# xmindflow/cenet

Measured on AMD Instinct MI355X. Metric: training images/sec (224x224, 4-class), higher is better.
Workload: dtype bf16

## Files before the change

### cenet_amd/csrc/common.h

```cpp
#pragma once

#ifdef CENET_HOSTSIM_BUILD
#include "hipsim.h"
#else
#include <hip/hip_runtime.h>
#include <cstdint>
#include <cstring>
typedef float f32x4 __attribute__((ext_vector_type(4)));
typedef float f32x16 __attribute__((ext_vector_type(16)));
typedef short bf16x8 __attribute__((ext_vector_type(8)));
#define CENET_LAUNCH(kernel, grid, block, stream, ...) \
  hipLaunchKernelGGL(kernel, (grid), (block), 0, (stream), __VA_ARGS__)
#endif

#define CENET_WAVE 64

struct cenet_bid {
  int x, y, z;
};
__device__ __forceinline__ cenet_bid cenet_xcd_block() {
  const int gx = gridDim.x, gy = gridDim.y;
  const int T = gx * gy * (int)gridDim.z;
  int L = blockIdx.x + gx * (blockIdx.y + gy * blockIdx.z);
  if (T >= 64) {
    const int per = T >> 3, rem = T & 7, xcd = L & 7, idx = L >> 3;
    L = xcd * per + (xcd < rem ? xcd : rem) + idx;
  }
  cenet_bid b;
  b.x = L % gx;
  const int t = L / gx;
  b.y = t % gy;
  b.z = t / gy;
  return b;
}

#ifdef CENET_HOSTSIM_BUILD
static const unsigned ring_zero16[4] = {0, 0, 0, 0};
#else
__device__ __attribute__((aligned(16))) const unsigned ring_zero16[4] = {0, 0, 0, 0};
#endif

__device__ __forceinline__ void ring_glds16(const void* gsrc, unsigned char* wave_base, int lane) {
#ifdef CENET_HOSTSIM_BUILD
  memcpy(wave_base + 16 * lane, gsrc, 16);
#else
  (void)lane;
  __builtin_amdgcn_global_load_lds((const __attribute__((address_space(1))) unsigned*)gsrc,
                                   (__attribute__((address_space(3))) unsigned*)wave_base, 16, 0, 0);
#endif
}

template <int N>
__device__ __forceinline__ void ring_wait_vm() {
#ifndef CENET_HOSTSIM_BUILD
  asm volatile("s_waitcnt vmcnt(%0)" ::"n"(N) : "memory");
#endif
}
__device__ __forceinline__ void ring_barrier() {
#ifdef CENET_HOSTSIM_BUILD
  __syncthreads();
#else
  asm volatile("s_barrier" ::: "memory");
#endif
}


#ifdef CENET_HOSTSIM_BUILD
__device__ __forceinline__ unsigned cenet_f2bf(float f) {
  unsigned u;
  memcpy(&u, &f, 4);
  u += 0x7FFFu + ((u >> 16) & 1u);
  return u >> 16;
}
__device__ __forceinline__ unsigned cenet_pack_bf2(float lo, float hi) { return cenet_f2bf(lo) | (cenet_f2bf(hi) << 16); }
#else
typedef __bf16 cenet_bf2_t __attribute__((ext_vector_type(2)));
__device__ __forceinline__ unsigned cenet_pack_bf2(float lo, float hi) {
  cenet_bf2_t v = {(__bf16)lo, (__bf16)hi};
  unsigned u;
  memcpy(&u, &v, 4);
  return u;
}
__device__ __forceinline__ unsigned cenet_f2bf(float f) { return cenet_pack_bf2(f, 0.f); }
#endif

typedef unsigned short bf16_t;
__device__ __forceinline__ float cenet_bf2f(unsigned h) {
  unsigned u = h << 16;
  float f;
  memcpy(&f, &u, 4);
  return f;
}
__device__ __forceinline__ float ldf(const float* p) { return *p; }
__device__ __forceinline__ float ldf(const bf16_t* p) { return cenet_bf2f(*p); }
__device__ __forceinline__ void stf(float* p, float v) { *p = v; }
__device__ __forceinline__ void stf(bf16_t* p, float v) { *p = (bf16_t)cenet_f2bf(v); }
struct f4 {
  float v[4];
};
__device__ __forceinline__ f4 ld4(const float* p) {
  f4 r;
  memcpy(r.v, p, 16);
  return r;
}
__device__ __forceinline__ f4 ld4(const bf16_t* p) {
  unsigned u[2];
  memcpy(u, p, 8);
  f4 r;
  r.v[0] = cenet_bf2f(u[0] & 0xFFFFu);
  r.v[1] = cenet_bf2f(u[0] >> 16);
  r.v[2] = cenet_bf2f(u[1] & 0xFFFFu);
  r.v[3] = cenet_bf2f(u[1] >> 16);
  return r;
}
__device__ __forceinline__ void st4(float* p, const f4& r) { memcpy(p, r.v, 16); }
// ... 244 lines not shown
```

### cenet_amd/csrc/gemm.hip

```cpp
#include "gemm_ring.h"
#include <cstdio>
#include <cstdlib>

static void pick_tile(int M, int N, int nbatch, int splits, int* bm, int* bn) {
  int m = M >= 96 ? 128 : (M >= 48 ? 64 : 32);
  int n = N >= 96 ? 128 : 64;
  if (m == 32) n = N >= 192 ? 256 : 64;
  long blocks = (long)cdiv(M, m) * cdiv(N, n) * nbatch * splits;
  if (blocks < 256 && m > 32) {
    int m2 = m > 64 ? 64 : m, n2 = n > 64 ? 64 : n;
    if (M >= 48) {
      m = m2;
      n = n2;
    }
  }
  *bm = m;
  *bn = n;
}

static thread_local char g_last_kernel[96] = "";
extern "C" const char* cenet_gemm_last_kernel(void) { return g_last_kernel; }
static inline const char* tf(bool b) { return b ? "true" : "false"; }

#ifdef CENET_RING_STAMPS
static unsigned long long* g_stamp_buf = nullptr;
static int g_stamp_n = 0;
extern "C" int cenet_ring_stamps(unsigned long long* buf, int n) {
  if (buf != nullptr && n <= 0) return CENET_EINVAL;
  g_stamp_buf = buf;
  g_stamp_n = buf ? n : 0;
  return CENET_OK;
}
#endif

template <typename GT>
__global__ __launch_bounds__(256) void gemm_asum_kernel(const GT* __restrict__ A, long sr, long sc, long skb, int M, int K, int nkb,
                                                       float* __restrict__ asum) {
  __shared__ float red[16];
  if (sr == 1 && sc != 1) {
    const int m = blockIdx.x * 256 + threadIdx.x;
    if (m >= M) return;
    const long total = (long)nkb * K;
    float s = 0.f;
    for (long e = blockIdx.y; e < total; e += gridDim.y) {
      const long kb = e / K, k = e - kb * K;
      s += ldf(A + kb * skb + k * sc + m);
    }
    atomicAdd(&asum[m], s);
  } else {
    const int m = blockIdx.x;
    const long total = (long)nkb * K;
    float s = 0.f;
    for (long e = blockIdx.y * 256 + threadIdx.x; e < total; e += (long)gridDim.y * 256) {
      const long kb = e / K, k = e - kb * K;
      s += ldf(A + kb * skb + (long)m * sr + k * sc);
    }
    s = block_sum(s, red);
    if (threadIdx.x == 0) atomicAdd(&asum[m], s);
  }
}
extern "C" int cenet_col_sum_acc_f32(const float* a, float* out_acc, long R, int C, hipStream_t stream);
extern "C" int cenet_col_sum_acc_bf16(const bf16_t* a, float* out_acc, long R, int C, hipStream_t stream);
extern "C" int cenet_chan_dot_acc_f32(const float* a, long sab, const float* b, long sbb, float* out_acc, int B, int C, int HW,
                                      hipStream_t stream);
extern "C" int cenet_chan_dot_acc_bf16(const bf16_t* a, long sab, const bf16_t* b, long sbb, float* out_acc, int B, int C, int HW,
                                       hipStream_t stream);

template <typename GT>
static void launch_asum(const cenet_mat_t* A, int M, int K, int nkb, float* asum, hipStream_t stream) {
  if (A->sr == 1 && A->sc == M && nkb == 1) {
    if (sizeof(GT) == 2) cenet_col_sum_acc_bf16((const bf16_t*)A->ptr, asum, K, M, stream);
    else cenet_col_sum_acc_f32((const float*)A->ptr, asum, K, M, stream);
    return;
  }
  if (A->sc == 1 && A->sr == K && (nkb == 1 || A->skb >= (long)M * K)) {
// ... 84 lines not shown
      g.b_end = (const unsigned short*)B->ptr + b_last;
      if (lda < 0 || ldb < 0 || a_last < 8 || b_last < 8) akf = bkf = -1;
    } else {
      akf = bkf = -1;
    }
  }
  static const bool ring_off = getenv("CENET_GEMM_NO_RING") != nullptr;
  const bool ring = !ring_off && akf >= 0 && bkf >= 0 && !E->cmode && E->act == ACT_NONE && M >= 48 && N >= 48;
  if (ring) {
    static const char* force = getenv("CENET_RING_TILE");
    if (force) {
      sscanf(force, "%dx%d", &bm, &bn);
    } else if (E->atomic) {
      bm = bn = 64;
      if ((long)K * nkb >= 4096 && (long)M * N >= 131072) {
        if (N >= 128) bn = 128;
        else bm = 128;
      }
    } else {
      bm = M >= 96 ? 128 : 64;
      bn = N >= 96 ? 128 : 64;
      const long want = K >= 320 ? 400 : 256;
      auto wgs = [&](int a, int b) { return (long)cdiv(M, a) * cdiv(N, b) * nbatch; };
      if (wgs(bm, bn) < want && bm == 128 && bn == 128) (M >= N ? bm : bn) = 64;
      if (wgs(bm, bn) < want && (bm == 128 || bn == 128)) bm = bn = 64;
      static const char* fb = getenv("CENET_RING_TILE_BATCHED");
      if (fb && nbatch >= 8) sscanf(fb, "%dx%d", &bm, &bn);
    }
  }
  const int kstep = ring ? 64 : BK;
  if (E->atomic && !E->cmode && splits > 1) {
    const long tiles = (long)cdiv(M, bm) * cdiv(N, bn) * nbatch;
    const long iters = (long)nkb * cdiv(K, kstep);
    const double t_iter = ring ? 0.5 : ((B->mode == 1) ? 2.0 : 0.9);
    const double t_atom = (double)tiles * bm * bn * 4.0 / 1.3e6;
    long s = (long)(__builtin_sqrt((double)iters * t_iter / t_atom) + 0.5);
    const long slots = (bm * bn >= 128 * 128) ? 512 : (bm * bn >= 128 * 64 ? 768 : 1024);
    if (s * tiles > slots) s = slots / tiles;
    if (s > iters / 2) s = iters / 2;
    if (s > 256) s = 256;
    if (s < 1) s = 1;
    static const char* sm = getenv("CENET_RING_SPLIT_MUL");
    if (ring && sm) {
      s = (long)(s * atof(sm) + 0.5);
      if (s > iters / 2) s = iters / 2;
      if (s < 1) s = 1;
    }
    splits = (int)s;
    g.splits = splits;
  }
  const bool im = B->mode != 0;
  int rc;
  static const bool stream_off = getenv("CENET_GEMM_NO_STREAM") != nullptr;
  const bool rstream = ring && !stream_off && !E->atomic && nkb == 1 && splits <= 1 && !g.ring_unal && (K == 64 || K == 128) &&
                       (long)cdiv(M, 64) * cdiv(N, 64) * nbatch >= 768;
  if (rstream) {
    snprintf(g_last_kernel, sizeof g_last_kernel, "gemm_ring_stream_kernel<%s, %s, %s, %d>", tf(akf), tf(bkf), tf(swap), K / 64);
    rc = akf ? (bkf ? cenet_gemm_launch_ring_kk(g, 0, 0, nbatch, swap, stream) : cenet_gemm_launch_ring_kr(g, 0, 0, nbatch, swap, stream))
             : (bkf ? cenet_gemm_launch_ring_rk(g, 0, 0, nbatch, swap, stream) : cenet_gemm_launch_ring_rr(g, 0, 0, nbatch, swap, stream));
  } else if (ring) {
    snprintf(g_last_kernel, sizeof g_last_kernel, "gemm_ring_kernel<%s, %s, %d, %d, %d, %s>", tf(akf), tf(bkf), bm, bn,
             bm == 128 && bn == 128 ? 2 : (bm == 64 && bn == 64 ? 4 : 3), tf(swap));
    rc = akf ? (bkf ? cenet_gemm_launch_ring_kk(g, bm, bn, nbatch, swap, stream) : cenet_gemm_launch_ring_kr(g, bm, bn, nbatch, swap, stream))
             : (bkf ? cenet_gemm_launch_ring_rk(g, bm, bn, nbatch, swap, stream) : cenet_gemm_launch_ring_rr(g, bm, bn, nbatch, swap, stream));
  } else if (bf) {
    if (E->asum) {
      launch_asum<unsigned short>(A, M, K, nkb, E->asum, stream);
      g.E.asum = nullptr;
    }
    const long kchunk = ((long)nkb * K) / (splits > 0 ? splits : 1);
    const bool k64 = !im && K >= 128 && kchunk >= 128 && bm <= 64 && bn == 64;
    snprintf(g_last_kernel, sizeof g_last_kernel, "gemm_kernel<unsigned short, %d, %d, %s, %s, %d>", bm, bn, tf(im), tf(swap),
             k64 ? 64 : 32);
    rc = im ? cenet_gemm_launch_bf16_im2col(g, bm, bn, nbatch, swap, stream)
            : (k64 ? cenet_gemm_launch_bf16_plain_k64(g, bm, bn, nbatch, swap, stream)
                   : cenet_gemm_launch_bf16_plain(g, bm, bn, nbatch, swap, stream));
  }
  else {
    if (E->asum) {
      launch_asum<float>(A, M, K, nkb, E->asum, stream);
      g.E.asum = nullptr;
    }
    snprintf(g_last_kernel, sizeof g_last_kernel, "gemm_kernel<float, %d, %d, %s, %s, 32>", bm, bn, tf(im), tf(swap));
    rc = im ? cenet_gemm_launch_f32_im2col(g, bm, bn, nbatch, swap, stream) : cenet_gemm_launch_f32_plain(g, bm, bn, nbatch, swap, stream);
  }
  if (rc != CENET_OK) return rc;
  CENET_CHECK_LAUNCH();
  return CENET_OK;
}

extern "C" int cenet_gemm_f32(const cenet_mat_t* A, const cenet_mat_t* B, const cenet_epi_t* E, int M, int N, int K,
                              int nbatch, int nb_inner, int nkb, int splits, hipStream_t stream) {
  return gemm_dispatch(A, B, E, M, N, K, nbatch, nb_inner, nkb, splits, 4, stream);
}
extern "C" int cenet_gemm_bf16(const cenet_mat_t* A, const cenet_mat_t* B, const cenet_epi_t* E, int M, int N, int K,
                               int nbatch, int nb_inner, int nkb, int splits, hipStream_t stream) {
  return gemm_dispatch(A, B, E, M, N, K, nbatch, nb_inner, nkb, splits, 2, stream);
}
```

### cenet_amd/csrc/gemm_core.h

```cpp
#pragma once
#include "common.h"
#include "../../include/cenet_hip.h"

struct GemmArgs {
  cenet_mat_t A, B;
  cenet_epi_t E;
  int M, N, K, nkb, splits, nb_inner;
  int avec, bvec, cvec;
  int cvec8;
  int apair, bpair;
  int ring_unal;
  const void *a_end, *b_end;
#ifdef CENET_RING_STAMPS
  unsigned long long* stamps;
  int stamp_n;
#endif
};

__device__ __forceinline__ unsigned f2bf_bits(float f) { return cenet_f2bf(f); }
__device__ __forceinline__ unsigned pack_bf2(float lo, float hi) { return cenet_pack_bf2(lo, hi); }

template <typename OpT, int KT> struct OpTraits { static constexpr int PITCH = KT + (sizeof(OpT) == 4 ? 4 : 8); };
#define BK 32

// ... 381 lines not shown
            const int row = SWAP ? rbase : rbase + r, col = SWAP ? cbase + r : cbase;
            if (row < g.M && col < g.N) {
              float t = v[r];
              if (E.bias) t += E.bias[E.bias_on_row ? row : col];
              t *= bsr > 0 ? E.bscale[row / bsr] : bs;
              if (Rb) t += ldf(Rb + (long)row * E.srr + (long)col * E.src);
              stf(Cb + (long)row * E.scr + (long)col * E.scc, t);
            }
          }
        }
      }
    return;
  }
  for (int f = 0; f < MI * NJ; ++f) {
    f32x4 t4 = acc[0][0];
#pragma unroll
    for (int i = 0; i < MI; ++i)
#pragma unroll
      for (int j = 0; j < NJ; ++j)
        if (f == i * NJ + j) t4 = acc[i][j];
    const int rbase = rwave + (f / NJ) * 16, cbase = cwave + (f % NJ) * 16;
#pragma unroll
    for (int r = 0; r < 4; ++r) {
      const int row = SWAP ? rbase : rbase + r, col = SWAP ? cbase + r : cbase;
      if (row < g.M && col < g.N) {
        float v = t4[r] * E.alpha;
        if (E.cmode) {
          const int kkw = E.cKH * E.cKW;
          const int ci = row / kkw, rem = row - ci * kkw;
          const int ky = rem / E.cKW, kx = rem - ky * E.cKW;
          const int py = col / E.cPw, px = col - py * E.cPw;
          const int iy = py * E.cstride - E.cpad + ky, ix = px * E.cstride - E.cpad + kx;
          if (iy >= 0 && iy < E.cHs && ix >= 0 && ix < E.cWs) {
            const long o = (long)ci * E.csci + (long)iy * E.csy + (long)ix * E.csx;
            if (E.atomic) atomicAdd(&Cf[o], v);
            else stf(&Cb[o], v);
          }
        } else if (E.atomic == 2) {
          Cf[(long)row * E.scr + (long)col * E.scc] = v;
        } else if (E.atomic) {
          atomicAdd(&Cf[(long)row * E.scr + (long)col * E.scc], v);
        } else {
          if (E.bias) v += E.bias[E.bias_on_row ? row : col];
          v = act_fwd(E.act, v, E.slope);
          v *= bsr > 0 ? E.bscale[row / bsr] : bs;
          if (Rb) v += ldf(Rb + (long)row * E.srr + (long)col * E.src);
          stf(&Cb[(long)row * E.scr + (long)col * E.scc], v);
        }
      }
    }
  }
}

template <typename OpT, int BM, int BN, bool B_IM2COL, bool SWAP, int KT>
__global__ __launch_bounds__(256, (BM * BN >= 128 * 128 ? 2 : 1)) void gemm_kernel(GemmArgs g) {
  static_assert(KT == 32 || (KT == 64 && !B_IM2COL), "K step: 32, or 64 for plain operands");
  constexpr int P = OpTraits<OpT, KT>::PITCH;
  constexpr bool BF = (sizeof(OpT) == 2);
  constexpr int MI = BM / 32, NJ = BN / 32;
  constexpr int NA = BM * KT / 256, NB = BN * KT / 256;
  typedef OpT GT;
  __shared__ __attribute__((aligned(16))) OpT As[BM * P];
  __shared__ __attribute__((aligned(16))) OpT Bs[BN * P];
  __shared__ KEntry ntab[B_IM2COL ? BN : 1];
  __shared__ float cstrip[SWAP ? 1 : 4 * 16 * (BN / 2 + 1)];

  const int tid = threadIdx.x, wave = tid >> 6, lane = tid & 63;
  const int wm = wave >> 1, wn = wave & 1;
  int bx, by, bz;
  {
    const int gx = gridDim.x, gy = gridDim.y;
    const int T = gx * gy * (int)gridDim.z;
    int L = blockIdx.x + gx * (blockIdx.y + gy * blockIdx.z);
    if (T >= 64) {
      const int per = T >> 3, rem = T & 7, xcd = L & 7, idx = L >> 3;
      L = xcd * per + (xcd < rem ? xcd : rem) + idx;
    }
    bx = L % gx;
    const int t = L / gx;
    by = t % gy;
    bz = t / gy;
  }
  const int batch = bz / g.splits, split = bz - batch * g.splits;
  const int bo = batch / g.nb_inner, bi = batch - bo * g.nb_inner;
  const int m0 = by * BM, n0 = bx * BN;

  f32x4 acc[MI][NJ];
#pragma unroll
  for (int i = 0; i < MI; ++i)
#pragma unroll
    for (int j = 0; j < NJ; ++j) acc[i][j] = f32x4{0.f, 0.f, 0.f, 0.f};

  const int ktiles = (g.K + KT - 1) / KT;
  const int total = g.nkb * ktiles;
  const int chunk = (total + g.splits - 1) / g.splits;
  const int it0 = split * chunk;
  const int it1 = (it0 + chunk < total) ? it0 + chunk : total;

  constexpr int A_KPT = KT / (256 / BM), B_KPT = KT / (256 / BN);
  static_assert(BM <= 256 && BN <= 256 && NA % 4 == 0 && NB % 4 == 0 && NA <= 64 && NB <= 64, "unsupported tile");
  StageRegs<NA> rga;
  StageRegs<NB> rgb;
  float* const ra = rga.f;
  float* const rb = rgb.f;
  const bool a_fast = g.A.kinner == 0, b_fast = !B_IM2COL && g.B.kinner == 0;
  const int avec = (g.avec == 8 && NA % 8 != 0) ? 4 : g.avec, bvec = (g.bvec == 8 && NB % 8 != 0) ? 4 : g.bvec;
// ... 275 lines not shown
```

### cenet_amd/csrc/gemm_ring.h

```cpp
#pragma once
#include "gemm_core.h"

typedef short ring_s4 __attribute__((ext_vector_type(4)));

__device__ __forceinline__ int kf_key(int row) { return (row >> 1) & 7; }
template <int BX>
__device__ __forceinline__ int rf_key(int k) {
  return BX == 128 ? 2 * (k & 3) + 8 * ((k >> 3) & 1) : 2 * ((k >> 1) & 1) + 4 * ((k >> 3) & 1);
}

__device__ __forceinline__ bf16x8 ring_frag_kf(const unsigned char* img, int r0, int kc, int lane) {
  const int row = r0 + (lane & 15), c = kc * 4 + (lane >> 4);
  bf16x8 f;
  memcpy(&f, img + (row * 8 + (c ^ kf_key(row))) * 16, 16);
  return f;
}
template <int BX>
__device__ __forceinline__ bf16x8 ring_frag_rf(const unsigned char* img, int r0, int kc, int lane) {
  constexpr int CH = BX / 8;
  const int g = lane >> 4, i = lane & 15;
  bf16x8 f;
#ifdef CENET_HOSTSIM_BUILD
  const int x = r0 + i;
#pragma unroll
  for (int j = 0; j < 8; ++j) {
    const int k = kc * 32 + 8 * g + j;
    const unsigned short* p = (const unsigned short*)(img + (k * CH + ((x >> 3) ^ rf_key<BX>(k))) * 16) + (x & 7);
    f[j] = (short)*p;
  }
#else
  const int q = i >> 2, p = i & 3;
  const int x = r0 + 4 * p;
#pragma unroll
  for (int h = 0; h < 2; ++h) {
    const int k = kc * 32 + 8 * g + 4 * h + q;
    const unsigned char* a = img + (k * CH + ((x >> 3) ^ rf_key<BX>(k))) * 16 + (x & 7) * 2;
    const ring_s4 v = __builtin_amdgcn_ds_read_tr16_b64_v4i16((ring_s4 __attribute__((address_space(3)))*)a);
    f[4 * h + 0] = v[0], f[4 * h + 1] = v[1], f[4 * h + 2] = v[2], f[4 * h + 3] = v[3];
  }
#endif
  return f;
}

template <int BX>
__device__ __forceinline__ bf16x8 ring_frag_rf_inflight(const unsigned char* img, int r0, int kc, int lane) {
#if defined(CENET_HOSTSIM_BUILD) || defined(CENET_RING_TR_BUILTIN)
  return ring_frag_rf<BX>(img, r0, kc, lane);
#else
  constexpr int CH = BX / 8;
  const int g = lane >> 4, i = lane & 15, q = i >> 2, p = i & 3;
  const int x = r0 + 4 * p;
  bf16x8 f;
#pragma unroll
  for (int h = 0; h < 2; ++h) {
    const int k = kc * 32 + 8 * g + 4 * h + q;
    const unsigned char* a = img + (k * CH + ((x >> 3) ^ rf_key<BX>(k))) * 16 + (x & 7) * 2;
    ring_s4 v;
    asm volatile("ds_read_b64_tr_b16 %0, %1"
                 : "=v"(v)
                 : "v"((unsigned)(__UINTPTR_TYPE__)(const __attribute__((address_space(3))) unsigned char*)a));
    f[4 * h + 0] = v[0], f[4 * h + 1] = v[1], f[4 * h + 2] = v[2], f[4 * h + 3] = v[3];
  }
  return f;
#endif
}
template <bool KF>
__device__ __forceinline__ void ring_frag_landed(bf16x8& f) {
#ifndef CENET_HOSTSIM_BUILD
  if (!KF) asm volatile("s_waitcnt lgkmcnt(0)" : "+v"(f));
#endif
}

template <int NI>
struct RingSrc {
  const bf16_t* p[NI];
  int kofs[NI];
};

template <bool KF, int BX>
__device__ __forceinline__ RingSrc<BX / 32> ring_src(const bf16_t* base, long ld, int x0, int X, int wave, int lane) {
  constexpr int NI = BX / 32, CH = BX / 8;
  RingSrc<NI> s;
#pragma unroll
  for (int j = 0; j < NI; ++j) {
    const int S = (j * 4 + wave) * 64 + lane;
    if (KF) {
      const int row = S >> 3, c = (S & 7) ^ kf_key(row);
      int r = x0 + row;
      r = r < X ? r : X - 1;
      s.p[j] = base + (long)r * ld + 8 * c;
      s.kofs[j] = 8 * c;
    } else {
      const int k = S / CH, c = (S % CH) ^ rf_key<BX>(k);
      int x = x0 + 8 * c;
      x = x < X ? x : x0;
      s.p[j] = base + (long)k * ld + x;
      s.kofs[j] = k;
    }
  }
  return s;
}

__device__ __forceinline__ void ring_fix_tail_chunk(const bf16_t* src, const bf16_t* end, unsigned char* slot) {
  const int d = (int)((src + 8) - end);
  unsigned short in[8], out[8];
#pragma unroll
  for (int j = 0; j < 8; ++j) in[j] = (end - 8)[j];
#pragma unroll
  for (int j = 0; j < 8; ++j) {
    unsigned short v = 0;
#pragma unroll
    for (int t = 1; t < 8; ++t)
      if (t == d && j + t < 8) v = in[j + t];
    out[j] = v;
  }
// ... 180 lines not shown
      for (int i = 0; i < MI; ++i) ring_frag_landed<AKF>(a[i]);
#pragma unroll
      for (int j = 0; j < NJ; ++j) ring_frag_landed<BKF>(b[j]);
      if (klim_t < 64) {
        if (AKF) {
#pragma unroll
          for (int i = 0; i < MI; ++i) a[i] = ring_mask_k(a[i], kc, lane, klim_t);
        }
        if (BKF) {
#pragma unroll
          for (int j = 0; j < NJ; ++j) b[j] = ring_mask_k(b[j], kc, lane, klim_t);
        }
      }
      if (do_asum) {
#pragma unroll
        for (int i = 0; i < MI; ++i)
#pragma unroll
          for (int j = 0; j < 8; ++j) rsum[i] += cenet_bf2f((unsigned short)a[i][j]);
      }
      clk.lap(RSEG_READS);
#pragma unroll
      for (int j = 0; j < NJ; ++j)
#pragma unroll
        for (int i = 0; i < MI; ++i)
          acc[i][j] = SWAP ? __builtin_amdgcn_mfma_f32_16x16x32_bf16(b[j], a[i], acc[i][j], 0, 0, 0)
                           : __builtin_amdgcn_mfma_f32_16x16x32_bf16(a[i], b[j], acc[i][j], 0, 0, 0);
      clk.lap(RSEG_MFMA);
    }
    if (t == 0) clk.first_step_done();
    cur = cur + 1 == NS ? 0 : cur + 1;
  }
  clk.store(g, blockIdx.x + gridDim.x * (blockIdx.y + gridDim.y * blockIdx.z), gridDim.x * gridDim.y * gridDim.z, T, tid);
  if (do_asum) {
#pragma unroll
    for (int i = 0; i < MI; ++i) {
      float v = rsum[i];
      v += __shfl_xor(v, 16);
      v += __shfl_xor(v, 32);
      const int row = m0 + wm * (BM / 2) + i * 16 + lane;
      if (lane < 16 && row < g.M) atomicAdd(&g.E.asum[row], v);
    }
  }
  __syncthreads();
  static_assert(NS * STAGE >= (BM > BN ? BM : BN) * ((BM > BN ? BN : BM) + 8) * 2 && NS * STAGE >= BM * (BN + 8) * 2,
                "the staged epilogue image reuses the ring");
  gemm_epilogue<bf16_t, BM, BN, SWAP, true>(g, acc, (float*)lds, m0, n0, bo, bi, batch, wave, lane);
}

template <bool AKF, bool BKF, bool SWAP, int T>
__global__ __launch_bounds__(256, 2) void gemm_ring_stream_kernel(GemmArgs g, int tiles_x, int tiles_y, int total_tiles) {
  constexpr int BM = 64, BN = 64, MI = 2, NJ = 2;
  constexpr int ABYTES = BM * 128, STAGE = (BM + BN) * 128;
  __shared__ __attribute__((aligned(1024))) unsigned char lds[2 * T * STAGE];
  const int tid = threadIdx.x, lane = tid & 63;
#ifdef CENET_HOSTSIM_BUILD
  const int wave = tid >> 6;
#else
  const int wave = __builtin_amdgcn_readfirstlane(tid >> 6);
#endif
  const int wm = wave >> 1, wn = wave & 1;
  const long lda = AKF ? g.A.sr : g.A.sc, ldb = BKF ? g.B.sc : g.B.sr;
  const long kstepA = AKF ? 1 : lda, kstepB = BKF ? 1 : ldb;
  auto tile_of = [&](int vt) -> int {
    if ((gridDim.x & 7) == 0 && total_tiles >= 64) {
      const int per = total_tiles >> 3, rem = total_tiles & 7, xcd = vt & 7, idx = vt >> 3;
      return xcd * per + (xcd < rem ? xcd : rem) + idx;
    }
    return vt;
  };
  struct Where { int m0, n0, bo, bi, batch; };
  auto where = [&](int L) -> Where {
    Where w;
    const int bx = L % tiles_x, t = L / tiles_x, by = t % tiles_y;
    w.batch = t / tiles_y;
    w.bo = w.batch / g.nb_inner;
    w.bi = w.batch - w.bo * g.nb_inner;
    w.m0 = by * BM;
    w.n0 = bx * BN;
    return w;
  };
  auto issue = [&](const Where& w, int set) __attribute__((always_inline)) {
    const bf16_t* baseA = (const bf16_t*)g.A.ptr + (long)w.bo * g.A.sb + (long)w.bi * g.A.sb2;
    const bf16_t* baseB = (const bf16_t*)g.B.ptr + (long)w.bo * g.B.sb + (long)w.bi * g.B.sb2;
    const RingSrc<MI> sa = ring_src<AKF, BM>(baseA, lda, w.m0, g.M, wave, lane);
    const RingSrc<NJ> sb = ring_src<BKF, BN>(baseB, ldb, w.n0, g.N, wave, lane);
#pragma unroll
    for (int kt = 0; kt < T; ++kt) {
      unsigned char* img = lds + (set * T + kt) * STAGE;
      ring_issue<AKF, BM>(sa, (long)kt * 64 * kstepA, 64, false, img, wave, lane, false, nullptr);
      ring_issue<BKF, BN>(sb, (long)kt * 64 * kstepB, 64, false, img + ABYTES, wave, lane, false, nullptr);
    }
  };
  int vt = blockIdx.x;
  if (vt >= total_tiles) return;
  Where cur = where(tile_of(vt));
  issue(cur, 0);
  ring_wait_vm<0>();
  RingClock clk;
  clk.start();
  int set = 0, trips = 0;
  for (; vt < total_tiles; vt += gridDim.x, set ^= 1, ++trips) {
    ring_barrier();
    clk.lap(RSEG_BARRIER);
    const int nvt = vt + gridDim.x;
    Where nxt = cur;
    if (nvt < total_tiles) {
      nxt = where(tile_of(nvt));
      issue(nxt, set ^ 1);
    }
    clk.lap(RSEG_ISSUE);
    f32x4 acc[MI][NJ];
#pragma unroll
    for (int i = 0; i < MI; ++i)
#pragma unroll
      for (int j = 0; j < NJ; ++j) acc[i][j] = f32x4{0.f, 0.f, 0.f, 0.f};
#pragma unroll
    for (int kt = 0; kt < T; ++kt) {
      const unsigned char* Ai = lds + (set * T + kt) * STAGE;
      const unsigned char* Bi = Ai + ABYTES;
#pragma unroll
      for (int kc = 0; kc < 2; ++kc) {
        bf16x8 a[MI], b[NJ];
#pragma unroll
        for (int i = 0; i < MI; ++i)
          a[i] = AKF ? ring_frag_kf(Ai, wm * 32 + i * 16, kc, lane) : ring_frag_rf_inflight<BM>(Ai, wm * 32 + i * 16, kc, lane);
#pragma unroll
        for (int j = 0; j < NJ; ++j)
          b[j] = BKF ? ring_frag_kf(Bi, wn * 32 + j * 16, kc, lane) : ring_frag_rf_inflight<BN>(Bi, wn * 32 + j * 16, kc, lane);
#pragma unroll
        for (int i = 0; i < MI; ++i) ring_frag_landed<AKF>(a[i]);
#pragma unroll
        for (int j = 0; j < NJ; ++j) ring_frag_landed<BKF>(b[j]);
        clk.lap(RSEG_READS);
#pragma unroll
        for (int j = 0; j < NJ; ++j)
#pragma unroll
          for (int i = 0; i < MI; ++i)
            acc[i][j] = SWAP ? __builtin_amdgcn_mfma_f32_16x16x32_bf16(b[j], a[i], acc[i][j], 0, 0, 0)
                             : __builtin_amdgcn_mfma_f32_16x16x32_bf16(a[i], b[j], acc[i][j], 0, 0, 0);
        clk.lap(RSEG_MFMA);
      }
    }
    ring_wait_vm<0>();
    clk.lap(RSEG_WAIT);
    gemm_epilogue<bf16_t, BM, BN, SWAP, false>(g, acc, (float*)nullptr, cur.m0, cur.n0, cur.bo, cur.bi, cur.batch, wave, lane);
    clk.lap(RSEG_REST);
    if (trips == 0) clk.first_step_done();
    cur = nxt;
  }
  clk.store(g, blockIdx.x, gridDim.x, trips, tid);
}

template <bool AKF, bool BKF, bool SWAP>
static int launch_ring_stream(const GemmArgs& g, int nbatch, hipStream_t stream) {
  const int tx = cdiv(g.N, 64), ty = cdiv(g.M, 64);
  const long total = (long)tx * ty * nbatch;
  if (total > (1L << 30)) return CENET_EUNSUPPORTED;
  static const char* ge = getenv("CENET_STREAM_WGS");
  long wgs = ge ? atol(ge) : 1024;
  if (wgs > total) wgs = total;
  if (wgs >= 8) wgs &= ~7L;
  if (g.K == 64) CENET_LAUNCH((gemm_ring_stream_kernel<AKF, BKF, SWAP, 1>), dim3((unsigned)wgs), dim3(256), stream, g, tx, ty, (int)total);
  else if (g.K == 128) CENET_LAUNCH((gemm_ring_stream_kernel<AKF, BKF, SWAP, 2>), dim3((unsigned)wgs), dim3(256), stream, g, tx, ty, (int)total);
  else return CENET_EUNSUPPORTED;
  return CENET_OK;
}

template <bool AKF, bool BKF, bool SWAP>
static int launch_ring(const GemmArgs& g, int bm, int bn, int nbatch, hipStream_t stream) {
  dim3 grid(cdiv(g.N, bn), cdiv(g.M, bm), nbatch * g.splits);
  if (grid.y > 65535 || grid.z > 65535) return CENET_EUNSUPPORTED;
  if (bm == 128 && bn == 128) {
    CENET_LAUNCH((gemm_ring_kernel<AKF, BKF, 128, 128, 2, SWAP>), grid, dim3(256), stream, g);
    return CENET_OK;
  }
  if (bm == 64 && bn == 64) {
    CENET_LAUNCH((gemm_ring_kernel<AKF, BKF, 64, 64, 4, SWAP>), grid, dim3(256), stream, g);
    return CENET_OK;
  }
  if (bm == 128 && bn == 64) {
    CENET_LAUNCH((gemm_ring_kernel<AKF, BKF, 128, 64, 3, SWAP>), grid, dim3(256), stream, g);
    return CENET_OK;
  }
  if (bm == 64 && bn == 128) {
    CENET_LAUNCH((gemm_ring_kernel<AKF, BKF, 64, 128, 3, SWAP>), grid, dim3(256), stream, g);
    return CENET_OK;
  }
  return CENET_EUNSUPPORTED;
}
#define CENET_RING_INSTANCE(NAME, AKF, BKF)                                                       \
  int NAME(const GemmArgs& g, int bm, int bn, int nbatch, bool swap, hipStream_t stream) {        \
    if (bm == 0)                                                                                  \
      return swap ? launch_ring_stream<AKF, BKF, true>(g, nbatch, stream)                         \
                  : launch_ring_stream<AKF, BKF, false>(g, nbatch, stream);                       \
    return swap ? launch_ring<AKF, BKF, true>(g, bm, bn, nbatch, stream)                          \
                : launch_ring<AKF, BKF, false>(g, bm, bn, nbatch, stream);                        \
  }
int cenet_gemm_launch_ring_kk(const GemmArgs& g, int bm, int bn, int nbatch, bool swap, hipStream_t stream);
int cenet_gemm_launch_ring_kr(const GemmArgs& g, int bm, int bn, int nbatch, bool swap, hipStream_t stream);
int cenet_gemm_launch_ring_rk(const GemmArgs& g, int bm, int bn, int nbatch, bool swap, hipStream_t stream);
int cenet_gemm_launch_ring_rr(const GemmArgs& g, int bm, int bn, int nbatch, bool swap, hipStream_t stream);
```

### cenet_amd/kern.py

```python
from __future__ import annotations

import ctypes as C
import math
from typing import Optional

import torch

from . import _lib
from ._lib import AttnT, DiffAttnT, EpiT, MatT, WgradProbT

ACT = {"none": 0, "relu": 1, "lrelu": 2, "gelu": 3, "silu": 4, "sigmoid": 5}


def _chk(*ts):
    for t in ts:
        if t is None:
            continue
        if isinstance(t, Ptr):
            t = t.t
        if t.dtype not in (torch.float32, torch.bfloat16, torch.int32, torch.int64, torch.uint8):
            raise TypeError(f"cenet_amd kernels take fp32 / bf16 tensors (int32 / int64 / uint8 for indices and masks); "
                            f"got {t.dtype}")
        if not t.is_cuda and not _lib.is_hostsim():
            raise RuntimeError("cenet_amd kernels run on the MI355X only: tensor is not on a CUDA/HIP device "
# ... 79 lines not shown
    e.bias_on_row = int(bias_on_row)
    e.act, e.slope = ACT[act], slope
    e.bscale = bscale.data_ptr() if bscale is not None else None
    e.bscale_rows = bscale_rows
    e.asum = asum.data_ptr() if asum is not None else None
    e.R = (R.data_ptr() + esz(R) * r_offset) if R is not None else None
    e.srb, e.srb2, e.srr, e.src = srb, srb2, srr, src
    e.atomic, e.alpha = int(atomic), alpha
    if col2im is not None:
        e.cmode = 1
        e.cKH, e.cKW, e.cPw = col2im["KH"], col2im["KW"], col2im["Pw"]
        e.cHs, e.cWs, e.cstride, e.cpad = col2im["Hs"], col2im["Ws"], col2im["stride"], col2im["pad"]
        e.csci, e.csy, e.csx = col2im["sci"], col2im["sy"], col2im["sx"]
    _launch("cenet_gemm_bf16" if A.bf16 else "cenet_gemm_f32", C.byref(A), C.byref(B), C.byref(e), M, N, K, nbatch, nb_inner, nkb,
            splits)


def _wgrad_array(probs):
    n = len(probs)
    arr = (WgradProbT * n)()
    for d, t in zip(arr, probs):
        d.A, d.B, d.C, d.asum, d.lda, d.ldb, d.skbA, d.skbB, d.M, d.N, d.K, d.nkb = t[:12]
        d.akf = d.bkf = t[12]
    return arr


def wgrad_group(probs, device, phases=(0,), between=None):
    n = len(probs)
    arr = _wgrad_array(probs)
    need = _lib.lib().cenet_wgrad_group_ws_floats(arr, n)
    ws = torch.empty(max(need, 1), device=device, dtype=torch.float32)
    for i, ph in enumerate(phases):
        if i and between is not None:
            between()
        if ph == 0:
            _launch("cenet_wgrad_group_bf16", arr, n, ws, need)
        else:
            _launch("cenet_wgrad_group_phase_bf16", arr, n, ws, need, ph)
    return need


def wgrad_group_plan(probs):
    n = len(probs)
    arr = _wgrad_array(probs)
    out = [(C.c_int * n)() for _ in range(4)]
    _lib.check(_lib.lib().cenet_wgrad_group_plan(arr, n, *out), "cenet_wgrad_group_plan")
    return [tuple(o[i] for o in out) for i in range(n)]


def last_gemm_kernel() -> str:
    return _lib.lib().cenet_gemm_last_kernel().decode()


def last_conv_kernel() -> str:
    return _lib.lib().cenet_conv_last_kernel().decode()


def last_norm_kernel() -> str:
    return _lib.lib().cenet_norm_last_kernel().decode()


class Ptr:

    def __init__(self, t, off: int = 0):
        self.t, self.off = t, off
        self.dtype = t.dtype

    def data_ptr(self):
        return self.t.data_ptr() + esz(self.t) * self.off


def _launch(name, *args):
    args = [a.data_ptr() if isinstance(a, (torch.Tensor, Ptr)) else a for a in args]
    _lib.check(getattr(_lib.lib(), name)(*args, stream()), name)


def _call(name, *args):
    cargs = []
    bf = False
    for a in args:
        if isinstance(a, (torch.Tensor, Ptr)):
            bf = bf or a.dtype == BF16
            a = a.data_ptr()
        cargs.append(a)
    if bf and not name.endswith("_bf16"):
        assert name.endswith("_f32"), name
        name = name[:-4] + "_bf16"
    _lib.check(getattr(_lib.lib(), name)(*cargs, stream()), name)


def flash_supported(D: int, Dv: int) -> bool:
    return bool(_lib.lib().cenet_flash_attn_supported(D, Dv))


def flashb_supported(D: int, Dv: int) -> bool:
    return D <= 64 and Dv <= 128


def flash_fwd(a: AttnT, bf16: bool = False):
    name = "cenet_flash_attn_fwd_bf16" if bf16 else "cenet_flash_attn_fwd_f32"
    _launch(name, C.byref(a))


def flash_bwd(a: AttnT, bf16: bool = False):
    name = "cenet_flash_attn_bwd_bf16" if bf16 else "cenet_flash_attn_bwd_f32"
    _launch(name, C.byref(a))
# ... 955 lines not shown
```

### include/cenet_hip.h

```cpp
#ifndef CENET_HIP_H
#define CENET_HIP_H

#ifdef __cplusplus
extern "C" {
#endif

#ifndef CENET_HOSTSIM_BUILD
typedef struct ihipStream_t* cenet_stream_t;
#else
typedef void* cenet_stream_t;
#endif

typedef struct {
  const void* ptr;
  long sb, sb2, skb, sr, sc;
  long sk_outer;
  int kinner;
  int mode, kfast;
  int patch_is_row, transposed;
  int KH, KW, Pw, Hs, Ws, stride, pad, dil;
  long sci, sy, sx;
} cenet_mat_t;

typedef struct {
  void* C;
  long scb, scb2, scr, scc;
  const float* bias;
  int bias_on_row;
  int act;
  float slope;
  const float* bscale;
  const void* R;
  long srb, srb2, srr, src;
  int atomic;
  float alpha;
  int cmode, cKH, cKW, cPw, cHs, cWs, cstride, cpad;
  long csci, csy, csx;
  int bscale_rows;
  float* asum;
} cenet_epi_t;

int cenet_gemm_f32(const cenet_mat_t* A, const cenet_mat_t* B, const cenet_epi_t* E, int M, int N, int K,
                   int nbatch, int nb_inner, int nkb, int splits, cenet_stream_t stream);
int cenet_gemm_bf16(const cenet_mat_t* A, const cenet_mat_t* B, const cenet_epi_t* E, int M, int N, int K,
                    int nbatch, int nb_inner, int nkb, int splits, cenet_stream_t stream);
const char* cenet_gemm_last_kernel(void);

typedef struct {
  const void* A;
  const void* B;
  float* C;
  float* asum;
  long lda, ldb, skbA, skbB;
  int M, N, K, nkb;
  int akf, bkf;
} cenet_wgrad_prob_t;
long cenet_wgrad_group_ws_floats(const cenet_wgrad_prob_t* p, int n);
int cenet_wgrad_group_bf16(const cenet_wgrad_prob_t* p, int n, float* ws, long ws_floats, cenet_stream_t stream);
int cenet_wgrad_group_plan(const cenet_wgrad_prob_t* p, int n, int* launch, int* bm, int* bn, int* ns);
int cenet_wgrad_group_phase_bf16(const cenet_wgrad_prob_t* p, int n, float* ws, long ws_floats, int phase, cenet_stream_t stream);

int cenet_conv_direct_supported(int Cin, int Cout, int k, int stride, int pad);
int cenet_conv_direct_bf16(const unsigned short* x, const float* w, unsigned short* y, int B, int Cin, int Cout, int H, int W,
                           int k, int dgrad, cenet_stream_t stream);
int cenet_conv_c1_supported(int Cin, int Cout, int k, int stride, int pad);
int cenet_pw_fewout_supported(int Cin, int Cout);
int cenet_pw_fewout_wgrad_supported(int Cin, int Cout);
int cenet_pw_fewout_fwd_bf16(const unsigned short* x, const unsigned short* W, const float* bias, unsigned short* y, int B, int Cin,
    int Cout, long HW, cenet_stream_t stream);
int cenet_pw_fewout_dgrad_bf16(const unsigned short* dy, const unsigned short* W, unsigned short* dx, int B, int Cin, int Cout,
    long HW, cenet_stream_t stream);
int cenet_pw_fewout_wgrad_bf16(const unsigned short* x, const unsigned short* dy, float* dW_acc, float* dbias_acc, int B, int Cin,
    int Cout, long HW, cenet_stream_t stream);
int cenet_pw_small_supported(int G);
int cenet_pw_small_bf16(const unsigned short* x, const unsigned short* W, unsigned short* y, int B, int groups, int G, long HW,
    int transpose, cenet_stream_t stream);
int cenet_conv_c1_fwd_bf16(const unsigned short* x, const float* w, unsigned short* y, int B, int Cout, int H, int W, int k,
    cenet_stream_t stream);
int cenet_conv_c1_wgrad_bf16(const unsigned short* x, const unsigned short* dy, float* dw_acc, int B, int Cout, int H, int W,
    int k, cenet_stream_t stream);
int cenet_conv_wgrad_direct_supported(int Cin, int Cout, int k, int stride, int pad);
long cenet_conv_wgrad_direct_ws_floats(int Cin, int Cout, int k);
int cenet_conv_wgrad_direct_bf16(const unsigned short* x, const unsigned short* dy, float* dw_acc, float* ws, int B, int Cin,
                                 int Cout, int H, int W, int k, cenet_stream_t stream);
const char* cenet_conv_last_kernel(void);

typedef struct {
  const void *q, *k, *v;
  void* o;
  float* lse;
  const void* dout;
  void *dq, *dk, *dv;
  float* delta;
  long qsb, qsh, qsi, qsd, ksb, ksh, ksi, ksd, vsb, vsh, vsi, vsd, osb, osh, osi, osd;
  int B, H, Nq, Nk, D, Dv, v_head_div;
  float scale;
  int dkv_zeroed;
  int dkv_f32;
  int finite_scores;
// ... 556 lines not shown
```

Before: 1900.

## Overlap stream-GEMM epilogue loads and stage output tile through LDS for coalesced stores

In the persistent ring stream GEMM kernel, bias, scale and residual operands for the current tile are now prefetched before the MFMA loop, so their latency hides behind compute. For full in-bounds tiles, the epilogue writes results into an LDS staging tile and then issues 16-byte coalesced global stores. It also waits only on the store count rather than draining all memory ops. The next-tile issue becomes unconditional, with a dummy zero-size issue on the last trip, and fragment reads always use the in-flight variant. This adds LDS usage and register pressure, which may lower occupancy. It also exposes runtime knobs for the workgroup count and the tile threshold.

```diff
diff --git a/cenet_amd/csrc/common.h b/cenet_amd/csrc/common.h
--- a/cenet_amd/csrc/common.h
+++ b/cenet_amd/csrc/common.h
@@ -36,8 +36,10 @@
 
 #ifdef CENET_HOSTSIM_BUILD
 static const unsigned ring_zero16[4] = {0, 0, 0, 0};
+static const float ring_one = 1.f;
 #else
 __device__ __attribute__((aligned(16))) const unsigned ring_zero16[4] = {0, 0, 0, 0};
+__device__ const float ring_one = 1.f;
 #endif
 
 __device__ __forceinline__ void ring_glds16(const void* gsrc, unsigned char* wave_base, int lane) {
@@ -56,11 +58,25 @@
   asm volatile("s_waitcnt vmcnt(%0)" ::"n"(N) : "memory");
 #endif
 }
+template <int N>
+__device__ __forceinline__ void ring_wait_vm_seen() {
+#ifndef CENET_HOSTSIM_BUILD
+  static_assert(N >= 0 && N <= 63, "vmcnt is six bits");
+  __builtin_amdgcn_s_waitcnt((N & 15) | ((N >> 4) << 14) | (7 << 4) | (15 << 8));
+#endif
+}
 __device__ __forceinline__ void ring_barrier() {
 #ifdef CENET_HOSTSIM_BUILD
   __syncthreads();
 #else
   asm volatile("s_barrier" ::: "memory");
+#endif
+}
+__device__ __forceinline__ void ring_barrier_lds() {
+#ifdef CENET_HOSTSIM_BUILD
+  __syncthreads();
+#else
+  asm volatile("s_waitcnt lgkmcnt(0)\n\ts_barrier" ::: "memory");
 #endif
 }
 
diff --git a/cenet_amd/csrc/gemm.hip b/cenet_amd/csrc/gemm.hip
--- a/cenet_amd/csrc/gemm.hip
+++ b/cenet_amd/csrc/gemm.hip
@@ -21,6 +21,13 @@
 static thread_local char g_last_kernel[96] = "";
 extern "C" const char* cenet_gemm_last_kernel(void) { return g_last_kernel; }
 static inline const char* tf(bool b) { return b ? "true" : "false"; }
+
+int g_cenet_stream_wgs = 0;
+extern "C" int cenet_gemm_stream_wgs(int n) {
+  if (n < 0) return CENET_EINVAL;
+  g_cenet_stream_wgs = n;
+  return CENET_OK;
+}
 
 #ifdef CENET_RING_STAMPS
 static unsigned long long* g_stamp_buf = nullptr;
@@ -211,8 +218,9 @@
   const bool im = B->mode != 0;
   int rc;
   static const bool stream_off = getenv("CENET_GEMM_NO_STREAM") != nullptr;
+  static const char* stream_min = getenv("CENET_STREAM_MIN_TILES");
   const bool rstream = ring && !stream_off && !E->atomic && nkb == 1 && splits <= 1 && !g.ring_unal && (K == 64 || K == 128) &&
-                       (long)cdiv(M, 64) * cdiv(N, 64) * nbatch >= 768;
+                       (long)cdiv(M, 64) * cdiv(N, 64) * nbatch >= (stream_min ? atol(stream_min) : 768);
   if (rstream) {
     snprintf(g_last_kernel, sizeof g_last_kernel, "gemm_ring_stream_kernel<%s, %s, %s, %d>", tf(akf), tf(bkf), tf(swap), K / 64);
     rc = akf ? (bkf ? cenet_gemm_launch_ring_kk(g, 0, 0, nbatch, swap, stream) : cenet_gemm_launch_ring_kr(g, 0, 0, nbatch, swap, stream))
diff --git a/cenet_amd/csrc/gemm_core.h b/cenet_amd/csrc/gemm_core.h
--- a/cenet_amd/csrc/gemm_core.h
+++ b/cenet_amd/csrc/gemm_core.h
@@ -457,6 +457,149 @@
   }
 }
 
+struct StreamEpiRegs {
+  float bb[2][4];
+  float rs[2][4];
+  unsigned long long rr[2][2];
+  float bs;
+};
+enum { STREAM_EPI_STORES = 2 };
+
+__device__ __forceinline__ float stream_ld_f32(const float* q) {
+#ifdef CENET_HOSTSIM_BUILD
+  return *q;
+#else
+  float v;
+  asm volatile("global_load_dword %0, %1, off" : "=v"(v) : "v"(q) : "memory");
+  return v;
+#endif
+}
+__device__ __forceinline__ unsigned long long stream_ld_b64(const void* q) {
+  unsigned long long v;
+#ifdef CENET_HOSTSIM_BUILD
+  memcpy(&v, q, 8);
+#else
+  asm volatile("global_load_dwordx2 %0, %1, off" : "=v"(v) : "v"(q) : "memory");
+#endif
+  return v;
+}
+
+template <bool SWAP>
+__device__ __forceinline__ void stream_epi_prefetch(const GemmArgs& g, StreamEpiRegs& p, bool live, int m0, int n0, int bo, int bi,
+                                                    int batch, int wave, int lane) {
+  const cenet_epi_t& E = g.E;
+  const int wm = wave >> 1, wn = wave & 1, fr = lane & 15, fq = lane >> 4;
+  const int rwave = m0 + wm * 32 + (SWAP ? fr : fq * 4);
+  const int cwave = n0 + wn * 32 + (SWAP ? fq * 4 : fr);
+  const int bsr = E.bscale ? E.bscale_rows : 0;
+  const float* one = &ring_one;
+  p.bs = stream_ld_f32((live && E.bscale && bsr == 0) ? E.bscale + batch : one);
+  {
+    const bool on = live && E.bias != nullptr;
+    const int along = (SWAP != (bool)E.bias_on_row) ? 1 : 0;
+    const float* b = on ? E.bias + (E.bias_on_row ? rwave : cwave) : one;
+    const int sx = on ? 16 : 0, sr = on ? along : 0;
+#pragma unroll
+    for (int x = 0; x < 2; ++x)
+#pragma unroll
+      for (int r = 0; r < 4; ++r) p.bb[x][r] = stream_ld_f32(b + sx * x + sr * r);
+  }
+  {
+    const float* q[2][4];
+#pragma unroll
+    for (int i = 0; i < 2; ++i)
+#pragma unroll
+      for (int r = 0; r < (SWAP ? 1 : 4); ++r) q[i][r] = one;
+    if (live && bsr > 0) {
+#pragma unroll
+      for (int i = 0; i < 2; ++i)
+#pragma unroll
+        for (int r = 0; r < (SWAP ? 1 : 4); ++r) q[i][r] = E.bscale + (rwave + 16 * i + r) / bsr;
+    }
+#pragma unroll
+    for (int i = 0; i < 2; ++i)
+#pragma unroll
+      for (int r = 0; r < (SWAP ? 1 : 4); ++r) p.rs[i][r] = stream_ld_f32(q[i][r]);
+  }
+  {
+    const bool on = live && E.R != nullptr;
+    const bf16_t* rrow = on ? (const bf16_t*)E.R + (long)bo * E.srb + (long)bi * E.srb2 + (long)rwave * E.srr + (long)cwave * E.src
+                            : (const bf16_t*)ring_zero16;
+    const long ri = on ? 16 * E.srr : 0, rj = on ? 16 * E.src : 0;
+#pragma unroll
+    for (int j = 0; j < 2; ++j)
+#pragma unroll
+      for (int i = 0; i < 2; ++i) p.rr[i][j] = stream_ld_b64(rrow + i * ri + j * rj);
+  }
+}
+
+template <bool SWAP, int N>
+__device__ __forceinline__ void stream_epi_landed(StreamEpiRegs& p) {
+#ifndef CENET_HOSTSIM_BUILD
+  asm volatile("s_waitcnt vmcnt(%[n])"
+               : "+v"(p.bs), "+v"(p.bb[0][0]), "+v"(p.bb[0][1]), "+v"(p.bb[0][2]), "+v"(p.bb[0][3]), "+v"(p.bb[1][0]),
+                 "+v"(p.bb[1][1]), "+v"(p.bb[1][2]), "+v"(p.bb[1][3])
+               : [n] "n"(N));
+  asm volatile("" : "+v"(p.rr[0][0]), "+v"(p.rr[0][1]), "+v"(p.rr[1][0]), "+v"(p.rr[1][1]), "+v"(p.rs[0][0]), "+v"(p.rs[1][0]));
+  if (!SWAP)
+    asm volatile("" : "+v"(p.rs[0][1]), "+v"(p.rs[0][2]), "+v"(p.rs[0][3]), "+v"(p.rs[1][1]), "+v"(p.rs[1][2]), "+v"(p.rs[1][3]));
+#endif
+}
+
+template <bool SWAP>
+__device__ __forceinline__ void stream_epi_finish(const GemmArgs& g, f32x4 (&acc)[2][2], const StreamEpiRegs& p, bf16_t* tile, int m0,
+                                                  int n0, int bo, int bi, int wave, int lane) {
+  constexpr int BI = 64, BO = 64, TP = BI + 8, CPR = BI / 8;
+  const cenet_epi_t& E = g.E;
+  const int wm = wave >> 1, wn = wave & 1, fr = lane & 15, fq = lane >> 4;
+  const int bsr = E.bscale ? E.bscale_rows : 0;
+  const float bs = p.bs, scale = E.alpha * bs;
+#pragma unroll
+  for (int j = 0; j < 2; ++j)
+#pragma unroll
+    for (int i = 0; i < 2; ++i) {
+      float v[4];
+#pragma unroll
+      for (int r = 0; r < 4; ++r) v[r] = acc[i][j][r];
+      if (E.bias) {
+#pragma unroll
+        for (int r = 0; r < 4; ++r) v[r] = v[r] * E.alpha + (E.bias_on_row ? p.bb[i][r] : p.bb[j][r]);
+#pragma unroll
+        for (int r = 0; r < 4; ++r) v[r] *= bs;
+      } else {
+#pragma unroll
+        for (int r = 0; r < 4; ++r) v[r] *= scale;
+      }
+      if (bsr > 0) {
+#pragma unroll
+        for (int r = 0; r < 4; ++r) v[r] *= p.rs[i][SWAP ? 0 : r];
+      }
+      if (E.R) {
+        const unsigned u0 = (unsigned)p.rr[i][j], u1 = (unsigned)(p.rr[i][j] >> 32);
+        v[0] += cenet_bf2f(u0 & 0xFFFFu), v[1] += cenet_bf2f(u0 >> 16);
+        v[2] += cenet_bf2f(u1 & 0xFFFFu), v[3] += cenet_bf2f(u1 >> 16);
+      }
+      const int in0 = (SWAP ? wn * 32 + j * 16 : wm * 32 + i * 16) + fq * 4;
+      const int out0 = (SWAP ? wm * 32 + i * 16 : wn * 32 + j * 16) + fr;
+      st4v(tile + out0 * TP + in0, v);
+    }
+  ring_barrier_lds();
+  const long so = SWAP ? E.scr : E.scc;
+  bf16_t* cb = (bf16_t*)E.C + (long)bo * E.scb + (long)bi * E.scb2 + (long)(SWAP ? m0 : n0) * so + (SWAP ? n0 : m0);
+  static_assert(BO * CPR == 256 * STREAM_EPI_STORES, "store instructions per wave and tile");
+  unsigned q[STREAM_EPI_STORES][4];
+#pragma unroll
+  for (int s = 0; s < STREAM_EPI_STORES; ++s) {
+    const int c = s * 256 + wave * 64 + lane;
+    memcpy(q[s], tile + (c / CPR) * TP + 8 * (c % CPR), 16);
+  }
+#pragma unroll
+  for (int s = 0; s < STREAM_EPI_STORES; ++s) {
+    const int c = s * 256 + wave * 64 + lane;
+    memcpy(cb + (long)(c / CPR) * so + 8 * (c % CPR), q[s], 16);
+  }
+}
+
 template <typename OpT, int BM, int BN, bool B_IM2COL, bool SWAP, int KT>
 __global__ __launch_bounds__(256, (BM * BN >= 128 * 128 ? 2 : 1)) void gemm_kernel(GemmArgs g) {
   static_assert(KT == 32 || (KT == 64 && !B_IM2COL), "K step: 32, or 64 for plain operands");
diff --git a/cenet_amd/csrc/gemm_ring.h b/cenet_amd/csrc/gemm_ring.h
--- a/cenet_amd/csrc/gemm_ring.h
+++ b/cenet_amd/csrc/gemm_ring.h
@@ -61,6 +61,17 @@
                  : "v"((unsigned)(__UINTPTR_TYPE__)(const __attribute__((address_space(3))) unsigned char*)a));
     f[4 * h + 0] = v[0], f[4 * h + 1] = v[1], f[4 * h + 2] = v[2], f[4 * h + 3] = v[3];
   }
+  return f;
+#endif
+}
+__device__ __forceinline__ bf16x8 ring_frag_kf_inflight(const unsigned char* img, int r0, int kc, int lane) {
+#ifdef CENET_HOSTSIM_BUILD
+  return ring_frag_kf(img, r0, kc, lane);
+#else
+  const int row = r0 + (lane & 15), c = kc * 4 + (lane >> 4);
+  const unsigned char* a = img + (row * 8 + (c ^ kf_key(row))) * 16;
+  bf16x8 f;
+  asm volatile("ds_read_b128 %0, %1" : "=v"(f) : "v"((unsigned)(__UINTPTR_TYPE__)(const __attribute__((address_space(3))) unsigned char*)a));
   return f;
 #endif
 }
@@ -347,6 +358,7 @@
   constexpr int BM = 64, BN = 64, MI = 2, NJ = 2;
   constexpr int ABYTES = BM * 128, STAGE = (BM + BN) * 128;
   __shared__ __attribute__((aligned(1024))) unsigned char lds[2 * T * STAGE];
+  __shared__ __attribute__((aligned(16))) bf16_t cimg[64 * (64 + 8)];
   const int tid = threadIdx.x, lane = tid & 63;
 #ifdef CENET_HOSTSIM_BUILD
   const int wave = tid >> 6;
@@ -355,6 +367,7 @@
 #endif
   const int wm = wave >> 1, wn = wave & 1;
   const long lda = AKF ? g.A.sr : g.A.sc, ldb = BKF ? g.B.sc : g.B.sr;
+  const bool stage_ok = g.cvec8 && g.cvec && !g.E.atomic && !g.E.cmode && g.E.act == ACT_NONE;
   const long kstepA = AKF ? 1 : lda, kstepB = BKF ? 1 : ldb;
   auto tile_of = [&](int vt) -> int {
     if ((gridDim.x & 7) == 0 && total_tiles >= 64) {
@@ -374,7 +387,7 @@
     w.n0 = bx * BN;
     return w;
   };
-  auto issue = [&](const Where& w, int set) __attribute__((always_inline)) {
+  auto issue = [&](const Where& w, int set, bool real) __attribute__((always_inline)) {
     const bf16_t* baseA = (const bf16_t*)g.A.ptr + (long)w.bo * g.A.sb + (long)w.bi * g.A.sb2;
     const bf16_t* baseB = (const bf16_t*)g.B.ptr + (long)w.bo * g.B.sb + (long)w.bi * g.B.sb2;
     const RingSrc<MI> sa = ring_src<AKF, BM>(baseA, lda, w.m0, g.M, wave, lane);
@@ -382,27 +395,28 @@
 #pragma unroll
     for (int kt = 0; kt < T; ++kt) {
       unsigned char* img = lds + (set * T + kt) * STAGE;
-      ring_issue<AKF, BM>(sa, (long)kt * 64 * kstepA, 64, false, img, wave, lane, false, nullptr);
-      ring_issue<BKF, BN>(sb, (long)kt * 64 * kstepB, 64, false, img + ABYTES, wave, lane, false, nullptr);
+      ring_issue<AKF, BM>(sa, (long)kt * 64 * kstepA, real ? 64 : 0, !real, img, wave, lane, false, nullptr);
+      ring_issue<BKF, BN>(sb, (long)kt * 64 * kstepB, real ? 64 : 0, !real, img + ABYTES, wave, lane, false, nullptr);
     }
   };
   int vt = blockIdx.x;
   if (vt >= total_tiles) return;
   Where cur = where(tile_of(vt));
-  issue(cur, 0);
-  ring_wait_vm<0>();
+  issue(cur, 0, true);
+  ring_wait_vm_seen<0>();
   RingClock clk;
   clk.start();
   int set = 0, trips = 0;
   for (; vt < total_tiles; vt += gridDim.x, set ^= 1, ++trips) {
     ring_barrier();
     clk.lap(RSEG_BARRIER);
+    const bool staged = stage_ok && cur.m0 + BM <= g.M && cur.n0 + BN <= g.N;
+    StreamEpiRegs er;
+    stream_epi_prefetch<SWAP>(g, er, staged, cur.m0, cur.n0, cur.bo, cur.bi, cur.batch, wave, lane);
     const int nvt = vt + gridDim.x;
-    Where nxt = cur;
-    if (nvt < total_tiles) {
-      nxt = where(tile_of(nvt));
-      issue(nxt, set ^ 1);
-    }
+    const bool more = nvt < total_tiles;
+    const Where nxt = where(tile_of(more ? nvt : vt));
+    issue(nxt, set ^ 1, more);
     clk.lap(RSEG_ISSUE);
     f32x4 acc[MI][NJ];
 #pragma unroll
@@ -418,14 +432,14 @@
         bf16x8 a[MI], b[NJ];
 #pragma unroll
         for (int i = 0; i < MI; ++i)
-          a[i] = AKF ? ring_frag_kf(Ai, wm * 32 + i * 16, kc, lane) : ring_frag_rf_inflight<BM>(Ai, wm * 32 + i * 16, kc, lane);
+          a[i] = AKF ? ring_frag_kf_inflight(Ai, wm * 32 + i * 16, kc, lane) : ring_frag_rf_inflight<BM>(Ai, wm * 32 + i * 16, kc, lane);
 #pragma unroll
         for (int j = 0; j < NJ; ++j)
-          b[j] = BKF ? ring_frag_kf(Bi, wn * 32 + j * 16, kc, lane) : ring_frag_rf_inflight<BN>(Bi, wn * 32 + j * 16, kc, lane);
-#pragma unroll
-        for (int i = 0; i < MI; ++i) ring_frag_landed<AKF>(a[i]);
-#pragma unroll
-        for (int j = 0; j < NJ; ++j) ring_frag_landed<BKF>(b[j]);
+          b[j] = BKF ? ring_frag_kf_inflight(Bi, wn * 32 + j * 16, kc, lane) : ring_frag_rf_inflight<BN>(Bi, wn * 32 + j * 16, kc, lane);
+#pragma unroll
+        for (int i = 0; i < MI; ++i) ring_frag_landed<false>(a[i]);
+#pragma unroll
+        for (int j = 0; j < NJ; ++j) ring_frag_landed<false>(b[j]);
         clk.lap(RSEG_READS);
 #pragma unroll
         for (int j = 0; j < NJ; ++j)
@@ -436,23 +450,32 @@
         clk.lap(RSEG_MFMA);
       }
     }
-    ring_wait_vm<0>();
-    clk.lap(RSEG_WAIT);
-    gemm_epilogue<bf16_t, BM, BN, SWAP, false>(g, acc, (float*)nullptr, cur.m0, cur.n0, cur.bo, cur.bi, cur.batch, wave, lane);
-    clk.lap(RSEG_REST);
+    stream_epi_landed<SWAP, 4 * T>(er);
+    if (staged) {
+      stream_epi_finish<SWAP>(g, acc, er, cimg, cur.m0, cur.n0, cur.bo, cur.bi, wave, lane);
+      clk.lap(RSEG_REST);
+      ring_wait_vm_seen<STREAM_EPI_STORES>();
+      clk.lap(RSEG_WAIT);
+    } else {
+      gemm_epilogue<bf16_t, BM, BN, SWAP, false>(g, acc, (float*)nullptr, cur.m0, cur.n0, cur.bo, cur.bi, cur.batch, wave, lane);
+      clk.lap(RSEG_REST);
+      ring_wait_vm_seen<0>();
+      clk.lap(RSEG_WAIT);
+    }
     if (trips == 0) clk.first_step_done();
     cur = nxt;
   }
   clk.store(g, blockIdx.x, gridDim.x, trips, tid);
 }
 
+extern int g_cenet_stream_wgs;
 template <bool AKF, bool BKF, bool SWAP>
 static int launch_ring_stream(const GemmArgs& g, int nbatch, hipStream_t stream) {
   const int tx = cdiv(g.N, 64), ty = cdiv(g.M, 64);
   const long total = (long)tx * ty * nbatch;
   if (total > (1L << 30)) return CENET_EUNSUPPORTED;
   static const char* ge = getenv("CENET_STREAM_WGS");
-  long wgs = ge ? atol(ge) : 1024;
+  long wgs = g_cenet_stream_wgs > 0 ? g_cenet_stream_wgs : (ge ? atol(ge) : 1024);
   if (wgs > total) wgs = total;
   if (wgs >= 8) wgs &= ~7L;
   if (g.K == 64) CENET_LAUNCH((gemm_ring_stream_kernel<AKF, BKF, SWAP, 1>), dim3((unsigned)wgs), dim3(256), stream, g, tx, ty, (int)total);
diff --git a/cenet_amd/kern.py b/cenet_amd/kern.py
--- a/cenet_amd/kern.py
+++ b/cenet_amd/kern.py
@@ -155,6 +155,10 @@
     return _lib.lib().cenet_gemm_last_kernel().decode()
 
 
+def gemm_stream_wgs(n: int = 0) -> None:
+    _lib.check(_lib.lib().cenet_gemm_stream_wgs(int(n)), "cenet_gemm_stream_wgs")
+
+
 def last_conv_kernel() -> str:
     return _lib.lib().cenet_conv_last_kernel().decode()
 
diff --git a/include/cenet_hip.h b/include/cenet_hip.h
--- a/include/cenet_hip.h
+++ b/include/cenet_hip.h
@@ -45,6 +45,7 @@
 int cenet_gemm_bf16(const cenet_mat_t* A, const cenet_mat_t* B, const cenet_epi_t* E, int M, int N, int K,
                     int nbatch, int nb_inner, int nkb, int splits, cenet_stream_t stream);
 const char* cenet_gemm_last_kernel(void);
+int cenet_gemm_stream_wgs(int n);
 
 typedef struct {
   const void* A;
```

Measured after the change: 1900. About the same (-0.0%).
